# leimao/Voice-Converter-CycleGAN

Hardware: NVIDIA H100
Metric: CycleGAN-VC train steps/sec @ batch 256x[24,128] MCEP (higher is better)
Workload: dtype f16f8 (forward / data gradient: fp16 MMA + two e4m3 cross-term MMAs = 2 MMA units per product; weight gradient: fp16 MMA alone, 1 unit; f32 accumulate)

## Files before the change

voice-converter-cyclegan_b200/csrc/tc_gemm.cu:

```cuda
#include "tc_gemm.cuh"
#include "geom.h"
#include "kernels.cuh"
#include "wgmma.cuh"

#include <cuda.h>
#include <stdint.h>
#include <stdio.h>
#include <string.h>

namespace {

typedef CUresult (*EncodeTiledFn)(CUtensorMap*, CUtensorMapDataType, cuuint32_t, void*, const cuuint64_t*, const cuuint64_t*,
                                  const cuuint32_t*, const cuuint32_t*, CUtensorMapInterleave, CUtensorMapSwizzle,
                                  CUtensorMapL2promotion, CUtensorMapFloatOOBfill);
EncodeTiledFn get_encoder() {
  static EncodeTiledFn fn = nullptr;
  if (!fn) {
    void* p = nullptr; cudaDriverEntryPointQueryResult q;
    if (cudaGetDriverEntryPoint("cuTensorMapEncodeTiled", &p, cudaEnableDefault, &q) == cudaSuccess && q == cudaDriverEntryPointSuccess)
      fn = (EncodeTiledFn)p;
  }
  return fn;
}
bool make_tmap3(CUtensorMap* m, const void* base, uint64_t d0, uint64_t d1, uint64_t d2, uint32_t b1) {
  EncodeTiledFn enc = get_encoder();
  if (!enc) return false;
  cuuint64_t dims[3] = {d0, d1, d2};
  cuuint64_t strides[2] = {d0 * 2, d0 * d1 * 2};
  cuuint32_t box[3] = {64, b1, 1};
  cuuint32_t es[3] = {1, 1, 1};
  return enc(m, CU_TENSOR_MAP_DATA_TYPE_BFLOAT16, 3, const_cast<void*>(base), dims, strides, box, es, CU_TENSOR_MAP_INTERLEAVE_NONE,
             CU_TENSOR_MAP_SWIZZLE_128B, CU_TENSOR_MAP_L2_PROMOTION_L2_256B, CU_TENSOR_MAP_FLOAT_OOB_FILL_NONE) == CUDA_SUCCESS;
}

bool make_tmap3_t(CUtensorMap* m, const void* base, CUtensorMapDataType dt, int esize, uint64_t d0, uint64_t d1, uint64_t d2, uint32_t b0, uint32_t b1) {
  EncodeTiledFn enc = get_encoder();
  if (!enc) return false;
  cuuint64_t dims[3] = {d0, d1, d2};
  cuuint64_t strides[2] = {d0 * (uint64_t)esize, d0 * d1 * (uint64_t)esize};
  cuuint32_t box[3] = {b0, b1, 1};
  cuuint32_t es[3] = {1, 1, 1};
  return enc(m, dt, 3, const_cast<void*>(base), dims, strides, box, es, CU_TENSOR_MAP_INTERLEAVE_NONE,
             b0 * esize == 64 ? CU_TENSOR_MAP_SWIZZLE_64B : CU_TENSOR_MAP_SWIZZLE_128B, CU_TENSOR_MAP_L2_PROMOTION_L2_256B,
             CU_TENSOR_MAP_FLOAT_OOB_FILL_NONE) == CUDA_SUCCESS;
}

__device__ __forceinline__ uint32_t smem_u32(const void* p) { return (uint32_t)__cvta_generic_to_shared(p); }

__device__ __forceinline__ void mbar_init(uint64_t* bar, uint32_t count) {
  asm volatile("mbarrier.init.shared::cta.b64 [%0], %1;" ::"r"(smem_u32(bar)), "r"(count));
}
__device__ __forceinline__ void fence_barrier_init() { asm volatile("fence.mbarrier_init.release.cluster;" ::: "memory"); }
__device__ __forceinline__ void mbar_wait(uint64_t* bar, uint32_t parity) {
  asm volatile(
      "{\n\t"
      ".reg .pred p;\n\t"
      "WAIT_LOOP:\n\t"
      "mbarrier.try_wait.parity.shared::cta.b64 p, [%0], %1;\n\t"
      "@p bra.uni WAIT_DONE;\n\t"
      "bra.uni WAIT_LOOP;\n\t"
      "WAIT_DONE:\n\t"
      "}" ::"r"(smem_u32(bar)), "r"(parity) : "memory");
}
__device__ __forceinline__ void cp_async16(uint32_t dst_smem, const void* src, uint32_t src_bytes) {
  asm volatile("cp.async.cg.shared.global [%0], [%1], 16, %2;" ::"r"(dst_smem), "l"(src), "r"(src_bytes) : "memory");
}
__device__ __forceinline__ void cp_async_arrive_noinc(uint64_t* bar) {
  asm volatile("cp.async.mbarrier.arrive.noinc.shared::cta.b64 [%0];" ::"r"(smem_u32(bar)) : "memory");
}
__device__ __forceinline__ void mbar_expect_tx(uint64_t* bar, uint32_t bytes) {
  asm volatile("mbarrier.arrive.expect_tx.shared::cta.b64 _, [%0], %1;" ::"r"(smem_u32(bar)), "r"(bytes) : "memory");
}
__device__ __forceinline__ void tma_load3(uint32_t dst_smem, const CUtensorMap* map, int c0, int c1, int c2, uint64_t* bar) {
  asm volatile("cp.async.bulk.tensor.3d.shared::cluster.global.tile.mbarrier::complete_tx::bytes [%0], [%1, {%2, %3, %4}], [%5];"
               ::"r"(dst_smem), "l"(map), "r"(c0), "r"(c1), "r"(c2), "r"(smem_u32(bar)) : "memory");
}
__device__ __forceinline__ void tma_prefetch_desc(const CUtensorMap* map) {
  asm volatile("prefetch.tensormap [%0];" ::"l"(map) : "memory");
}
__device__ __forceinline__ void fence_proxy_async() { asm volatile("fence.proxy.async.shared::cta;" ::: "memory"); }
__device__ __forceinline__ uint64_t make_desc(uint32_t smem_addr, uint32_t lbo_bytes, uint32_t sbo_bytes, uint64_t layout = 1) {
  return (uint64_t)((smem_addr >> 4) & 0x3FFF) | ((uint64_t)((lbo_bytes >> 4) & 0x3FFF) << 16) |
         ((uint64_t)((sbo_bytes >> 4) & 0x3FFF) << 32) | (layout << 62);
}
__device__ __forceinline__ uint64_t make_desc64(uint32_t smem_addr) { return make_desc(smem_addr, 16, 512, 2); }
template <int N>
__device__ __forceinline__ void fence_acc(float (&d)[N]) {
#pragma unroll
  for (int i = 0; i < N; ++i) asm volatile("" : "+f"(d[i])::"memory");
}
__device__ __forceinline__ void mbar_arrive(uint64_t* bar) {
  asm volatile("mbarrier.arrive.shared::cta.b64 _, [%0];" ::"r"(smem_u32(bar)) : "memory");
}
__device__ __forceinline__ void consumer_bar() { asm volatile("bar.sync 3, 256;" ::: "memory"); }
__device__ __forceinline__ void st_shared16(uint32_t addr, uint4 v) {
  asm volatile("st.shared.v4.b32 [%0], {%1, %2, %3, %4};" ::"r"(addr), "r"(v.x), "r"(v.y), "r"(v.z), "r"(v.w) : "memory");
}
__device__ __forceinline__ uint4 e4m3x8_to_f16x8(uint2 v) {
  uint32_t w[4];
#pragma unroll
  for (int i = 0; i < 4; ++i) {
    const uint32_t src = (i < 2 ? v.x : v.y) >> (16 * (i & 1));
    const __half2_raw h = __nv_cvt_fp8x2_to_halfraw2((__nv_fp8x2_storage_t)(src & 0xFFFFu), __NV_E4M3);
    w[i] = (uint32_t)h.x | ((uint32_t)h.y << 16);
  }
  return make_uint4(w[0], w[1], w[2], w[3]);
}

struct FastDiv { uint32_t mul, shr, d; };
__host__ inline FastDiv make_fastdiv(uint32_t d) {
  FastDiv f; f.d = d;
  uint32_t l = 0; while ((1ull << l) < d) ++l;
  f.mul = (uint32_t)(((1ull << 32) * ((1ull << l) - d)) / d + 1);
  f.shr = l;
  return f;
}
__device__ __forceinline__ uint32_t fdiv(uint32_t n, const FastDiv& f) { return (uint32_t)(((uint64_t)__umulhi(n, f.mul) + n) >> f.shr); }

__device__ __forceinline__ uint32_t sw128(int r, int c) { return (uint32_t)((r >> 3) * 1024 + (r & 7) * 128 + ((c ^ (r & 7)) << 4)); }

struct TcNTParams {
  GatherGeom g;
  const __nv_bfloat16 *a_hi, *a_lo; int a_ld; int C;
  const __nv_bfloat16 *b_hi, *b_lo; int Nw;
  int N;
  int n_tiles;
  int debug;
  float* dst; int d_ld; const float* bias; int accumulate;
  int perm; int Cc;
  int R;
  const float *gamma_a, *beta_a, *gamma_g, *beta_g;
  float* stats;
  const float* resid;
  float* y; __nv_bfloat16 *y_hi, *y_lo;
  int C_out;
  const float* bp; int bp_ld;
  __nv_bfloat16 *dp_hi, *dp_lo; int dp_ld;
  float *dbeta_a, *dgamma_a, *dbeta_g, *dgamma_g;
  CUtensorMap tm_b_hi, tm_b_lo;
  const uint8_t *a8_hi, *a8_lo;
  CUtensorMap tm_b8_hi, tm_b8_lo;
  uint8_t* y8;
  PackGeom pk;
  FastDiv div_bw, div_w;
};

struct RowPos { int b, y, x; };
__device__ __forceinline__ RowPos nt_row(const TcNTParams& p, long long m) {
  RowPos r;
  r.y = (int)fdiv((uint32_t)m, p.div_bw);
  const uint32_t rem = (uint32_t)m - (uint32_t)r.y * p.div_bw.d;
  r.b = (int)fdiv(rem, p.div_w);
  r.x = (int)(rem - (uint32_t)r.b * p.div_w.d);
  return r;
}
template <int PK = 0>
__device__ __forceinline__ uint32_t nt_tile_taps(const TcNTParams& p, long long m0, long long M) {
  const long long m1 = m0 + 127 < M ? m0 + 127 : M - 1;
  if constexpr (PK == 2) {
    const int dout = p.pk.div * p.g.sx;
    const Pack2Pos a = pack2_pos(p.pk, p.g.Hy, dout, m0), b = pack2_pos(p.pk, p.g.Hy, dout, m1);
    return a.u == b.u ? gather_tap_mask(p.g, a.y, b.y) : (1u << p.g.ntaps) - 1u;
  }
  return gather_tap_mask(p.g, nt_row(p, m0).y, nt_row(p, m1).y);
}

struct TcTNParams {
  GatherGeom g;
  const __nv_bfloat16 *x_hi, *x_lo; int x_ld; int C;
  const __nv_bfloat16 *g_hi, *g_lo; int g_ld; int N;
  float* dw_a; float* dw_g; int n_split;
  int ksplit;
  FastDiv div_hw, div_w;
  CUtensorMap tm_g_hi, tm_g_lo;
  const uint8_t *x8_hi, *x8_lo;
  const uint8_t *g8_hi, *g8_lo;
  int w16;
  int fold_n;
  float* part; long long part_k, numel_a;
  PackGeom pk;
};

__device__ __forceinline__ float* tn_dst(float* base, int slab, int C, int c, int ncols, int col, int fold_n) {
  if (fold_n) { const int t = col / fold_n; return base + ((long long)t * C + c) * fold_n + (col - t * fold_n); }
  return base + ((long long)slab * C + c) * ncols + col;
}

constexpr int kProducerThreads = 128;


template <int BN, int NPL>
struct NTCfg {
  static constexpr int A_PLANE = 128 * 128;
  static constexpr int B_PLANE = BN * 128;
  static constexpr int PLANES = NPL == 2 ? 2 : 1;
  static constexpr int STAGE = PLANES * (A_PLANE + B_PLANE);
  static constexpr int STAGES = (192 * 1024) / STAGE;
  static constexpr int SMEM = STAGES * STAGE + 1024;
// ... 394 lines not shown
        }
        float t[32];
#pragma unroll
        for (int k = 0; k < 32; ++k) t[k] = dy[k];
        float s1a = warp_colsum32(t, lane);
#pragma unroll
        for (int k = 0; k < 32; ++k) t[k] = dy[k] * xa[k];
        float s2a = warp_colsum32(t, lane);
        float s1g = 0.f, s2g = 0.f;
        if (EPI == 3) {
#pragma unroll
          for (int k = 0; k < 32; ++k) t[k] = dg[k];
          s1g = warp_colsum32(t, lane);
#pragma unroll
          for (int k = 0; k < 32; ++k) t[k] = dg[k] * xg[k];
          s2g = warp_colsum32(t, lane);
        }
        if (p.dbeta_a && live) {
          atomicAdd(p.dbeta_a + ch + lane, s1a); atomicAdd(p.dgamma_a + ch + lane, s2a);
          if (EPI == 3) { atomicAdd(p.dbeta_g + ch + lane, s1g); atomicAdd(p.dgamma_g + ch + lane, s2g); }
        }
        s1a = sample_sum(s1a, epi_xch, q, lane, spw, barid); s2a = sample_sum(s2a, epi_xch, q, lane, spw, barid);
        if (EPI == 3) { s1g = sample_sum(s1g, epi_xch, q, lane, spw, barid); s2g = sample_sum(s2g, epi_xch, q, lane, spw, barid); }
        {
          const float sca = bc[64 + lane], scg = EPI == 3 ? bc[192 + lane] : 0.f;
          __syncwarp();
          bc[256 + lane] = sca * s1a * invR; bc[288 + lane] = sca * s2a * invR;
          if (EPI == 3) { bc[320 + lane] = scg * s1g * invR; bc[352 + lane] = scg * s2g * invR; }
          __syncwarp();
        }
#pragma unroll
        for (int k = 0; k < 32; k += 4) {
          float c1[4], c2[4], c3[4];
          bc4(bc + 64 + k, c1); bc4(bc + 256 + k, c2); bc4(bc + 288 + k, c3);
#pragma unroll
          for (int j = 0; j < 4; ++j) dy[k + j] = fmaf(c1[j], dy[k + j], -fmaf(xa[k + j], c3[j], c2[j]));
        }
        hwrite_y(stg, dy, nullptr, p.dp_hi, p.dp_lo, mq, M, p.dp_ld, ch, lane);
        if (EPI == 3) {
#pragma unroll
          for (int k = 0; k < 32; k += 4) {
            float c1[4], c2[4], c3[4];
            bc4(bc + 192 + k, c1); bc4(bc + 320 + k, c2); bc4(bc + 352 + k, c3);
#pragma unroll
            for (int j = 0; j < 4; ++j) dg[k + j] = fmaf(c1[j], dg[k + j], -fmaf(xg[k + j], c3[j], c2[j]));
          }
          hwrite_y(stg, dg, nullptr, p.dp_hi, p.dp_lo, mq, M, p.dp_ld, C + ch, lane);
        }
      }
    }
  }
}

enum { MMA_BF16 = 0, MMA_BF16X3 = 1, MMA_E4M3_CROSS = 2, MMA_F16 = 3, MMA_F16_CROSS = 4 };

template <int BN, int KIND, int TN, class Cfg>
__device__ __forceinline__ void consume_stages(float (&d)[BN / 2], int nkb, int& stage, uint32_t& phase, int& prev,
                                               uint64_t* full_bar, uint64_t* empty_bar, uint32_t smem_base, int wg, int lane) {
  for (int kb = 0; kb < nkb; ++kb) {
    mbar_wait(&full_bar[stage], phase);
    fence_proxy_async();
    const uint32_t sA = smem_base + stage * Cfg::STAGE + wg * 8192;
    const uint32_t sB = smem_base + stage * Cfg::STAGE + Cfg::PLANES * Cfg::A_PLANE;
    fence_acc(d);
    wgmma_fence();
    if constexpr (TN == 0) {
      if constexpr (KIND == MMA_E4M3_CROSS) {
#pragma unroll
        for (int k = 0; k < 2; ++k) {
          wgmma_e4m3<BN>(d, make_desc(sA + k * 32, 16, 1024), make_desc64(sB + Cfg::B_PLANE / 2 + k * 32), 1);
          wgmma_e4m3<BN>(d, make_desc(sA + 64 + k * 32, 16, 1024), make_desc64(sB + k * 32), 1);
        }
      } else if constexpr (KIND == MMA_F16) {
#pragma unroll
        for (int k = 0; k < 4; ++k)
          wgmma_f16<BN, 0, 0>(d, make_desc(sA + k * 32, 16, 1024), make_desc(sB + k * 32, 16, 1024), 1);
      } else {
#pragma unroll
        for (int k = 0; k < 4; ++k) {
          const uint64_t a_hi = make_desc(sA + k * 32, 16, 1024), b_hi = make_desc(sB + k * 32, 16, 1024);
          wgmma_bf16<BN, 0, 0>(d, a_hi, b_hi, 1);
          if constexpr (KIND == MMA_BF16X3) {
            const uint64_t a_lo = make_desc(sA + Cfg::A_PLANE + k * 32, 16, 1024), b_lo = make_desc(sB + Cfg::B_PLANE + k * 32, 16, 1024);
            wgmma_bf16<BN, 0, 0>(d, a_hi, b_lo, 1);
            wgmma_bf16<BN, 0, 0>(d, a_lo, b_hi, 1);
          }
        }
      }
    } else {
#pragma unroll
      for (int k = 0; k < 4; ++k) {
        const uint64_t a0 = make_desc(sA + k * 2048, 8192, 1024), b0 = make_desc(sB + k * 2048, 8192, 1024);
        const uint64_t a1 = make_desc(sA + Cfg::A_PLANE + k * 2048, 8192, 1024), b1 = make_desc(sB + Cfg::B_PLANE + k * 2048, 8192, 1024);
        if constexpr (KIND == MMA_F16_CROSS) {
          wgmma_f16<BN, 1, 1>(d, a0, b1, 1);
          wgmma_f16<BN, 1, 1>(d, a1, b0, 1);
        } else if constexpr (KIND == MMA_F16) {
          wgmma_f16<BN, 1, 1>(d, a0, b0, 1);
        } else {
          wgmma_bf16<BN, 1, 1>(d, a0, b0, 1);
          if constexpr (KIND == MMA_BF16X3) {
            wgmma_bf16<BN, 1, 1>(d, a0, b1, 1);
            wgmma_bf16<BN, 1, 1>(d, a1, b0, 1);
          }
        }
      }
    }
    wgmma_commit();
    wgmma_wait<1>();
    fence_acc(d);
    if (prev >= 0 && lane == 0) mbar_arrive(&empty_bar[prev]);
    prev = stage;
    if (++stage == Cfg::STAGES) { stage = 0; phase ^= 1; }
  }
}
template <int N>
__device__ __forceinline__ void rescale_acc(float (&d)[N], float scale) {
  wgmma_wait<0>();
  fence_acc(d);
#pragma unroll
  for (int i = 0; i < N; ++i) d[i] *= scale;
}

template <int BN, int PK = 0>
__device__ __forceinline__ void nt_store_fragments(const TcNTParams& p, const float (&d)[BN / 2], const long long M,
                                                   const long long m0, const int n0, const int r, const int c) {
  const GatherGeom& g = p.g;
  float* rowp[2];
#pragma unroll
  for (int h = 0; h < 2; ++h) {
    const long long m = m0 + r + 8 * h;
    rowp[h] = nullptr;
    if (m < M && p.dst) {
      if constexpr (PK == 2) {
        const int dout = p.pk.div * g.sx;
        const Pack2Pos o = pack2_pos(p.pk, g.Hy, dout, m);
        const long long r = pack2_row(o.o0, o.o1, g.Hd, dout / g.dsx, o.y * g.dsy + g.doy, o.x * g.dsx + g.dox);
        if (r >= 0) rowp[h] = p.dst + r * p.d_ld;
      } else {
        const RowPos o = nt_row(p, m);
        rowp[h] = p.dst + ((long long)(o.b * g.Hd + o.y * g.dsy + g.doy) * g.Wd + o.x * g.dsx + g.dox) * p.d_ld;
      }
    }
  }
  const bool vec = (p.d_ld & 1) == 0;
#pragma unroll
  for (int j = 0; j < BN / 8; ++j) {
    const int cb = j >> 2;
    const int n = (p.perm == 2 ? (cb >> 2) * p.Cc + ((cb >> 1) & 1) * (p.Cc >> 1) + (n0 >> 2) + (cb & 1) * 32
                   : p.perm    ? ((cb < 4) ? (n0 >> 1) + cb * 32 : p.Cc + (n0 >> 1) + (cb - 4) * 32) : n0 + cb * 32) + ((8 * j) & 31) + c;
    if (n >= p.N) continue;
    float2 bb = make_float2(0.f, 0.f);
    if (p.bias) bb = *reinterpret_cast<const float2*>(p.bias + n0 + 8 * j + c);
#pragma unroll
    for (int h = 0; h < 2; ++h) {
      float* rp = rowp[h];
      if (rp == nullptr) continue;
      float v0 = d[4 * j + 2 * h], v1 = d[4 * j + 2 * h + 1];
      if (p.bias) { v0 += bb.x; v1 += bb.y; }
      if (vec && n + 2 <= p.N) {
        if (p.accumulate)
          asm volatile("red.global.add.v2.f32 [%0], {%1, %2};" ::"l"(rp + n), "f"(v0), "f"(v1) : "memory");
        else
          *reinterpret_cast<float2*>(rp + n) = make_float2(v0, v1);
      } else {
        if (p.accumulate) atomicAdd(rp + n, v0); else rp[n] = v0;
        if (n + 1 < p.N) { if (p.accumulate) atomicAdd(rp + n + 1, v1); else rp[n + 1] = v1; }
      }
    }
  }
}

constexpr int kNTThreads = 384;

template <int BN, int NPL, int EPI, int PK = 0>
__global__ void __launch_bounds__(kNTThreads, 1)
tc_gg_nt_kernel(const __grid_constant__ TcNTParams p) {
  static_assert(!PK || EPI == 0, "packed rows never take the fused epilogues (they need whole equal-length samples per tile)");
  using Cfg = NTCfg<BN, NPL>;
  __shared__ float epi_xch[2][4][32];
  __shared__ __align__(16) float epi_bc[8][(EPI == 3 || EPI == 4) ? 384 : 128];
  __shared__ __align__(16) float epi_stage[8][32 * 16];
  __shared__ float* epi_rowp[8][32];
  constexpr int S = Cfg::STAGES;
  extern __shared__ uint8_t smem_raw[];
  __shared__ __align__(8) uint64_t full_bar[S], empty_bar[S], acc_free_bar;

  const uint32_t smem_base = (smem_u32(smem_raw) + 1023u) & ~1023u;
  const int warp = threadIdx.x >> 5, lane = threadIdx.x & 31;
  const GatherGeom& g = p.g;
  const long long M = (long long)g.B * g.Hy * g.Wx;
  const int cchunks = p.C >> 6;
  const int m_tiles = (int)((M + 127) / 128);
  const int n_tiles = p.n_tiles;
  const int num_tiles = m_tiles * n_tiles;
  const bool n_fast = g.Hy > 1;

  if (threadIdx.x == 0) {
    for (int s = 0; s < S; ++s) { mbar_init(&full_bar[s], kProducerThreads + 1); mbar_init(&empty_bar[s], 8); }
    mbar_init(&acc_free_bar, 8);
    fence_barrier_init();
    tma_prefetch_desc(&p.tm_b_hi);
    if (NPL == 2) tma_prefetch_desc(&p.tm_b_lo);
    if (NPL == 3) { tma_prefetch_desc(&p.tm_b8_hi); tma_prefetch_desc(&p.tm_b8_lo); }
  }
  __syncthreads();

  if (warp < 4) {
    const int t = threadIdx.x;
    const int chunk = t & 7, rsub = t >> 3;
    int stage = 0; uint32_t phase = 0;
    int it = 0;
    for (int tile = blockIdx.x; tile < num_tiles; tile += gridDim.x, ++it) {
      const long long m0 = (long long)(n_fast ? tile / n_tiles : tile % m_tiles) * 128;
      const int n0 = (n_fast ? tile % n_tiles : tile / m_tiles) * BN;
      if (EPI != 0 && it > 0) mbar_wait(&acc_free_bar, (uint32_t)(it - 1) & 1u);
      const uint32_t taps = nt_tile_taps<PK>(p, m0, M);
      int rb[8], ry[8], rx[8];
      int rw[PK == 2 ? 8 : 1];
#pragma unroll
      for (int i = 0; i < 8; ++i) {
        long long m = m0 + rsub + 16 * i;
        if (m < M) {
          if constexpr (PK == 2) {
            const Pack2Pos o = pack2_pos(p.pk, g.Hy, p.pk.div * g.sx, m);
            rb[i] = (int)(g.Hs * o.o0 / p.pk.div); rw[i] = (int)((o.o1 - o.o0) / p.pk.div); ry[i] = o.y * g.sy; rx[i] = o.x * g.sx;
          } else if constexpr (PK) {
            const int dout = p.pk.div * g.sx;
            const int u = pack_find(p.pk.off, p.pk.n, m * dout);
            const long long o0 = __ldg(p.pk.off + u), o1 = __ldg(p.pk.off + u + 1);
            rb[i] = (int)(o0 / p.pk.div); ry[i] = (int)((o1 - o0) / p.pk.div); rx[i] = (int)(m - o0 / dout) * g.sx;
          } else {
            const RowPos o = nt_row(p, m);
            rb[i] = o.b; ry[i] = o.y * g.sy; rx[i] = o.x * g.sx;
          }
        } else { rb[i] = -1; ry[i] = 0; rx[i] = 0; }
      }
      for (int pass = 0; pass < (NPL == 3 ? 2 : 1); ++pass)
      for (int tap = 0; tap < g.ntaps; ++tap) {
        if (!((taps >> tap) & 1u)) continue;
        long long aoff[8];
#pragma unroll
        for (int i = 0; i < 8; ++i) {
          const int cofs = NPL == 3 && pass == 0 ? (chunk & 3) * 16 : chunk * 8;
          if constexpr (PK == 2) {
            const int yy = ry[i] + g.oy[tap], xx = rx[i] + g.ox[tap];
            aoff[i] = rb[i] >= 0 && yy >= 0 && yy < g.Hs && xx >= 0 && xx < rw[i] ? ((long long)rb[i] + yy * rw[i] + xx) * p.a_ld + cofs : -1;
          } else if constexpr (PK) {
            const int xx = rx[i] + g.ox[tap];
            aoff[i] = rb[i] >= 0 && xx >= 0 && xx < ry[i] ? (long long)(rb[i] + xx) * p.a_ld + cofs : -1;
          } else {
            int yy = ry[i] + g.oy[tap], xx = rx[i] + g.ox[tap];
            bool ok = rb[i] >= 0 && yy >= 0 && yy < g.Hs && xx >= 0 && xx < g.Ws;
            aoff[i] = ok ? ((long long)(rb[i] * g.Hs + yy) * g.Ws + xx) * p.a_ld + cofs : -1;
          }
        }
        for (int cc = 0; cc < cchunks; ++cc) {
          const int c0 = cc << 6;
          mbar_wait(&empty_bar[stage], phase ^ 1);
          const uint32_t sA = smem_base + stage * Cfg::STAGE;
          const uint32_t sB = sA + Cfg::PLANES * Cfg::A_PLANE;
          if (t == 0) {
            mbar_expect_tx(&full_bar[stage], Cfg::PLANES * Cfg::B_PLANE);
            if (NPL == 3) {
              if (pass == 0) {
                tma_load3(sB, &p.tm_b8_hi, c0, n0, g.widx[tap], &full_bar[stage]);
                tma_load3(sB + Cfg::B_PLANE / 2, &p.tm_b8_lo, c0, n0, g.widx[tap], &full_bar[stage]);
              } else {
                tma_load3(sB, &p.tm_b_hi, c0, n0, g.widx[tap], &full_bar[stage]);
              }
            } else {
              tma_load3(sB, &p.tm_b_hi, c0, n0, g.widx[tap], &full_bar[stage]);
              if (NPL == 2) tma_load3(sB + Cfg::B_PLANE, &p.tm_b_lo, c0, n0, g.widx[tap], &full_bar[stage]);
            }
          }
          if (!(p.debug & 4)) {
#pragma unroll
            for (int i = 0; i < 8; ++i) {
              const int r = rsub + 16 * i;
              const uint32_t so = sw128(r, chunk);
              const bool ok = aoff[i] >= 0;
              const long long off = ok ? aoff[i] + c0 : 0;
              if (NPL == 3) {
                if (pass == 0)
                  cp_async16(sA + so, (chunk < 4 ? p.a8_hi : p.a8_lo) + off, ok ? 16u : 0u);
                else
                  cp_async16(sA + so, p.a_hi + off, ok ? 16u : 0u);
              } else {
                cp_async16(sA + so, p.a_hi + off, ok ? 16u : 0u);
                if (NPL == 2) cp_async16(sA + Cfg::A_PLANE + so, p.a_lo + off, ok ? 16u : 0u);
              }
            }
          }
          cp_async_arrive_noinc(&full_bar[stage]);
          if (++stage == S) { stage = 0; phase ^= 1; }
        }
      }
    }
  } else {
    const int cw = warp - 4;
    const int wg = cw >> 2;
    const int tw = threadIdx.x - 128 * (wg + 1);
    float* acc_s = reinterpret_cast<float*>(smem_raw + (smem_base - smem_u32(smem_raw)));
    int stage = 0; uint32_t phase = 0;
    for (int tile = blockIdx.x; tile < num_tiles; tile += gridDim.x) {
      const long long m0 = (long long)(n_fast ? tile / n_tiles : tile % m_tiles) * 128;
      const int n0 = (n_fast ? tile % n_tiles : tile / m_tiles) * BN;
      float d[BN / 2];
#pragma unroll
      for (int i = 0; i < BN / 2; ++i) d[i] = 0.f;
      int prev = -1;
      const int kb_pass = __popc(nt_tile_taps<PK>(p, m0, M)) * cchunks;
      if constexpr (NPL == 3) {
        consume_stages<BN, MMA_E4M3_CROSS, 0, Cfg>(d, kb_pass, stage, phase, prev, full_bar, empty_bar, smem_base, wg, lane);
        rescale_acc(d, 1.f / (float)(1 << CGVC_Q_ACC_SHIFT));
        consume_stages<BN, MMA_F16, 0, Cfg>(d, kb_pass, stage, phase, prev, full_bar, empty_bar, smem_base, wg, lane);
      } else {
        consume_stages<BN, NPL == 2 ? MMA_BF16X3 : MMA_BF16, 0, Cfg>(d, kb_pass, stage, phase, prev, full_bar, empty_bar, smem_base, wg, lane);
      }
      wgmma_wait<0>();
      fence_acc(d);
      if (prev >= 0 && lane == 0) mbar_arrive(&empty_bar[prev]);
      const int r0 = wg * 64 + (tw >> 5) * 16 + ((tw & 31) >> 2), c0 = 2 * (tw & 3);
      if constexpr (EPI == 0) {
        if (!(p.debug & 3)) nt_store_fragments<BN, PK>(p, d, M, m0, n0, r0, c0);
      } else {
        consumer_bar();
        if (!(p.debug & 2)) {
#pragma unroll
          for (int j = 0; j < BN / 8; ++j) {
            *reinterpret_cast<float2*>(acc_s + acc_off<BN>(r0, 8 * j + c0)) = make_float2(d[4 * j], d[4 * j + 1]);
            *reinterpret_cast<float2*>(acc_s + acc_off<BN>(r0 + 8, 8 * j + c0)) = make_float2(d[4 * j + 2], d[4 * j + 3]);
          }
        }
        consumer_bar();
        nt_tile_epilogue<BN, NPL, EPI>(p, M, m0, n0, cw & 3, lane, epi_stage[cw], epi_rowp[cw], epi_bc[cw], epi_xch[wg], acc_s, wg, 2);
        fence_proxy_async();
        __syncwarp();
        if (lane == 0) mbar_arrive(&acc_free_bar);
      }
    }
  }
}

#define CGVC_Q_WGRAD_SHIFT 12
template <int NPL, int W16>
struct TNCfg {
  static constexpr int A_PLANE = 64 * 256;
  static constexpr int B_PLANE = 64 * 512;
  static constexpr int PLANES = (NPL == 1 || W16) ? 1 : 2;
  static constexpr int STAGE = PLANES * (A_PLANE + B_PLANE);
  static constexpr int STAGES = (192 * 1024) / STAGE;
  static constexpr int SMEM = STAGES * STAGE + 1024;
};

template <int NPL, int W16, int DET, int PK = 0>
__global__ void __launch_bounds__(kNTThreads, 1)
tc_gg_tn_kernel(const __grid_constant__ TcTNParams p) {
  static_assert(W16 == 0 || NPL == 3, "the fp16-only weight gradient is a form of CGVC_PREC_F16F8");
  using Cfg = TNCfg<NPL, W16>;
  constexpr int S = Cfg::STAGES;
  constexpr int BN = 256;
  extern __shared__ uint8_t smem_raw[];
  __shared__ __align__(8) uint64_t full_bar[S], empty_bar[S];

  const uint32_t smem_base = (smem_u32(smem_raw) + 1023u) & ~1023u;
  const int warp = threadIdx.x >> 5, lane = threadIdx.x & 31;
// ... 302 lines not shown
  {
    const int lane = t & 31, warp = t >> 5;
    const int cig = (lane & 3) * 8;
    const int col = warp * 8 + (lane >> 2);
    const int co = co0 + col;
    if (co < J.cout && ci0 + cig < J.cin_q) {
      float va[4], vb[4];
#pragma unroll
      for (int k = 0; k < 4; ++k) { va[k] = tile[cig + k][col]; vb[k] = tile[cig + 4 + k][col]; }
      const int nrow = perm_row(J.perm, co, J.cout, J.noff);
      const long long o = ((long long)tap * J.nt_n + nrow) * J.cin_q + ci0 + cig;
      uint2 ha, hb; uint32_t a_hi, a_lo, b_hi, b_lo;
      cgvc_quant4(va, CGVC_Q_W_SHI, CGVC_Q_W_SLO, ha, a_hi, a_lo);
      cgvc_quant4(vb, CGVC_Q_W_SHI, CGVC_Q_W_SLO, hb, b_hi, b_lo);
      *reinterpret_cast<uint4*>(J.q16 + o) = make_uint4(ha.x, ha.y, hb.x, hb.y);
      *reinterpret_cast<uint2*>(J.q8hi + o) = make_uint2(a_hi, b_hi);
      *reinterpret_cast<uint2*>(J.q8lo + o) = make_uint2(a_lo, b_lo);
    }
  }
  if (tap == 0 && tci == 0 && tco == 0 && J.b_off >= 0)
    for (int i = t; i < J.cout; i += 256) J.bias[perm_row(J.perm, i, J.cout, J.noff)] = params[J.b_off + i];
}

template <class K>
cudaError_t set_smem(K kernel, int bytes) {
  static std::vector<const void*> done;
  const void* key = (const void*)kernel;
  for (const void* d : done) if (d == key) return cudaSuccess;
  cudaError_t e = cudaFuncSetAttribute(kernel, cudaFuncAttributeMaxDynamicSharedMemorySize, bytes);
  if (e == cudaSuccess) done.push_back(key);
  return e;
}

struct ProfRec { cudaEvent_t a, b; double flops; int cls; long long M; int N, K; };
bool g_prof_on = false;
std::vector<ProfRec> g_prof;
void prof_begin(cudaStream_t st, double flops, int cls, long long M = 0, int N = 0, int K = 0) {
  if (!g_prof_on) return;
  ProfRec r; r.flops = flops; r.cls = cls; r.M = M; r.N = N; r.K = K;
  cudaEventCreate(&r.a); cudaEventCreate(&r.b);
  cudaEventRecord(r.a, st);
  g_prof.push_back(r);
}
void prof_end(cudaStream_t st) { if (g_prof_on && !g_prof.empty()) cudaEventRecord(g_prof.back().b, st); }

inline int tile_rows(int n_real, int n_padded) { return (n_padded % 256 == 0) ? 256 : (n_real <= 32 ? 32 : 128); }

int num_sms() {
  static int n = 0;
  if (!n) { int dev = 0; cudaGetDevice(&dev); cudaDeviceGetAttribute(&n, cudaDevAttrMultiProcessorCount, dev); }
  return n;
}

cudaError_t launch_nt(TcNTParams p, int precision, cudaStream_t st, int epi) {
  const long long M = (long long)p.g.B * p.g.Hy * p.g.Wx;
  if (M == 0) return cudaSuccess;
  if (M >= (1ll << 31)) return cudaErrorInvalidValue;
  const bool x3 = precision == 1;
  if (p.g.ntaps == 0) return cudaErrorInvalidValue;
  p.div_bw = make_fastdiv((uint32_t)(p.g.B * p.g.Wx)); p.div_w = make_fastdiv((uint32_t)p.g.Wx);
  const int bn = tile_rows(p.N, p.Nw);
  p.n_tiles = bn == 32 ? 1 : p.Nw / bn;
  const long long tiles = ((M + 127) / 128) * p.n_tiles;
  dim3 grid((unsigned)(tiles < num_sms() ? tiles : num_sms()));
  cudaError_t e;
  ++g_cgvc_launches;
  prof_begin(st, 2.0 * (double)M * p.N * p.g.ntaps * p.C, (epi == 1 || epi == 2 || epi == 5) ? 2 : 0, M, p.N, p.g.ntaps * p.C);
#define LAUNCH_NT(BN_, NPL_, EPI_, ...)                                                                        \
  do {                                                                                                         \
    e = set_smem(tc_gg_nt_kernel<BN_, NPL_, EPI_, ##__VA_ARGS__>, NTCfg<BN_, NPL_>::SMEM);                     \
    if (e != cudaSuccess) return e;                                                                            \
    tc_gg_nt_kernel<BN_, NPL_, EPI_, ##__VA_ARGS__><<<grid, kNTThreads, NTCfg<BN_, NPL_>::SMEM, st>>>(p);      \
  } while (0)
  if (epi != 0 && bn != 256) return cudaErrorInvalidValue;
  if (p.pk.off && (p.g.Hy > 1 || p.g.Hs > 1 || p.g.Hd > 1)) {
    if (epi != 0 || p.g.B != 1 || p.g.ntaps > 31) return cudaErrorInvalidValue;
    const int npl = precision == 3 ? 3 : x3 ? 2 : 1;
    if (bn == 256)      { if (npl == 3) LAUNCH_NT(256, 3, 0, 2); else if (npl == 2) LAUNCH_NT(256, 2, 0, 2); else LAUNCH_NT(256, 1, 0, 2); }
    else if (bn == 128) { if (npl == 3) LAUNCH_NT(128, 3, 0, 2); else if (npl == 2) LAUNCH_NT(128, 2, 0, 2); else LAUNCH_NT(128, 1, 0, 2); }
    else                { if (npl == 3) LAUNCH_NT(32, 3, 0, 2);  else if (npl == 2) LAUNCH_NT(32, 2, 0, 2);  else LAUNCH_NT(32, 1, 0, 2); }
  }
  else if (p.pk.off) {
    if (epi != 0 || p.g.B != 1 || p.g.Hy != 1) return cudaErrorInvalidValue;
    const int npl = precision == 3 ? 3 : x3 ? 2 : 1;
    if (bn == 256)      { if (npl == 3) LAUNCH_NT(256, 3, 0, 1); else if (npl == 2) LAUNCH_NT(256, 2, 0, 1); else LAUNCH_NT(256, 1, 0, 1); }
    else if (bn == 128) { if (npl == 3) LAUNCH_NT(128, 3, 0, 1); else if (npl == 2) LAUNCH_NT(128, 2, 0, 1); else LAUNCH_NT(128, 1, 0, 1); }
    else                { if (npl == 3) LAUNCH_NT(32, 3, 0, 1);  else if (npl == 2) LAUNCH_NT(32, 2, 0, 1);  else LAUNCH_NT(32, 1, 0, 1); }
  }
  else if (precision == 3) {
    if (epi == 1)       LAUNCH_NT(256, 3, 1);
    else if (epi == 2)  LAUNCH_NT(256, 3, 2);
    else if (epi == 5)  LAUNCH_NT(256, 3, 5);
    else if (epi != 0)  return cudaErrorInvalidValue;
    else if (bn == 256) LAUNCH_NT(256, 3, 0);
    else if (bn == 128) LAUNCH_NT(128, 3, 0);
    else                LAUNCH_NT(32, 3, 0);
  }
  else if (epi == 1)  { if (x3) LAUNCH_NT(256, 2, 1); else LAUNCH_NT(256, 1, 1); }
  else if (epi == 2)  { if (x3) LAUNCH_NT(256, 2, 2); else LAUNCH_NT(256, 1, 2); }
  else if (epi == 3)  { if (x3) LAUNCH_NT(256, 2, 3); else LAUNCH_NT(256, 1, 3); }
  else if (epi == 4)  { if (x3) LAUNCH_NT(256, 2, 4); else LAUNCH_NT(256, 1, 4); }
  else if (epi == 5)  { if (x3) LAUNCH_NT(256, 2, 5); else LAUNCH_NT(256, 1, 5); }
  else if (bn == 256) { if (x3) LAUNCH_NT(256, 2, 0); else LAUNCH_NT(256, 1, 0); }
  else if (bn == 128) { if (x3) LAUNCH_NT(128, 2, 0); else LAUNCH_NT(128, 1, 0); }
  else                { if (x3) LAUNCH_NT(32, 2, 0);  else LAUNCH_NT(32, 1, 0); }
#undef LAUNCH_NT
  prof_end(st);
  return cudaGetLastError();
}

cudaError_t launch_tn(TcTNParams p, int precision, cudaStream_t st, const DetSlab* det) {
  const long long M = (long long)p.g.B * p.g.Hy * p.g.Wx;
  if (M == 0) return cudaSuccess;
  if (M >= (1ll << 31)) return cudaErrorInvalidValue;
  const int tiles = ((p.g_ld + 255) / 256) * ((p.x_ld + 127) / 128) * p.g.ntaps;
  const int nsm = num_sms();
  long long maxsplit = M / 1024; if (maxsplit < 1) maxsplit = 1; if (maxsplit > 32) maxsplit = 32;
  int ksplit = 1; double best = 0.0;
  for (int ks = 1; ks <= (int)maxsplit; ++ks) {
    long long items = (long long)tiles * ks;
    double eff = (double)items / (double)(((items + nsm - 1) / nsm) * nsm);
    if (items < nsm) eff *= 0.5;
    if (eff > best + 0.02) { best = eff; ksplit = ks; }
  }
  const long long numel = (long long)p.g.ntaps * p.C * p.N;
  auto chunk_of = [&](int ks) { return ((M + ks - 1) / ks + 63) / 64 * 64; };
  if (det && det->p)
    while (ksplit > 1 && ((long long)ksplit * numel > det->cap || (long long)(ksplit - 1) * chunk_of(ksplit) >= M)) --ksplit;
  const bool det_split = det && det->p && ksplit > 1;
  if (det_split) { p.part = det->p; p.part_k = numel; p.numel_a = (long long)p.g.ntaps * p.C * p.n_split; }
  p.ksplit = ksplit;
  p.div_hw = make_fastdiv((uint32_t)(p.g.Hy * p.g.Wx)); p.div_w = make_fastdiv((uint32_t)p.g.Wx);
  const long long items = (long long)tiles * ksplit;
  dim3 grid((unsigned)(items < nsm ? items : nsm));
  cudaError_t e;
  ++g_cgvc_launches;
  prof_begin(st, 2.0 * (double)M * p.N * p.g.ntaps * p.C, 1, M, p.N, p.g.ntaps * p.C);
#define LAUNCH_TN(NPL_, W16_, DET_, ...)                                                                      \
  do {                                                                                                        \
    e = set_smem(tc_gg_tn_kernel<NPL_, W16_, DET_, ##__VA_ARGS__>, TNCfg<NPL_, W16_>::SMEM);                  \
    if (e != cudaSuccess) return e;                                                                           \
    tc_gg_tn_kernel<NPL_, W16_, DET_, ##__VA_ARGS__><<<grid, kNTThreads, TNCfg<NPL_, W16_>::SMEM, st>>>(p);   \
  } while (0)
  if (p.pk.off && (p.g.Hy > 1 || p.g.Hs > 1)) {
    if (p.g.B != 1) return cudaErrorInvalidValue;
    if (det_split) {
      if (precision == 3) { if (p.w16) LAUNCH_TN(3, 1, 1, 2); else LAUNCH_TN(3, 0, 1, 2); }
      else if (precision == 1) LAUNCH_TN(2, 0, 1, 2);
      else                     LAUNCH_TN(1, 0, 1, 2);
    } else {
      if (precision == 3) { if (p.w16) LAUNCH_TN(3, 1, 0, 2); else LAUNCH_TN(3, 0, 0, 2); }
      else if (precision == 1) LAUNCH_TN(2, 0, 0, 2);
      else                     LAUNCH_TN(1, 0, 0, 2);
    }
  } else if (p.pk.off) {
    if (p.g.B != 1 || p.g.Hy != 1) return cudaErrorInvalidValue;
    if (det_split) {
      if (precision == 3) { if (p.w16) LAUNCH_TN(3, 1, 1, 1); else LAUNCH_TN(3, 0, 1, 1); }
// ... 231 lines not shown
    L.bias = (float*)p; p += rnd((size_t)nt_n(L) * sizeof(float));
    if (!make_layer_maps(L)) return (int)cudaErrorInvalidValue;
    L.wq16 = nullptr; L.wq8hi = L.wq8lo = nullptr; L.wdq16 = nullptr; L.wdq8hi = L.wdq8lo = nullptr;
    if (w.quant && layer_ok_q(L)) {
      L.wq16 = p; p += rnd(wq_elems(L) * 2);
      L.wq8hi = (uint8_t*)p; p += rnd(wq_elems(L)); L.wq8lo = (uint8_t*)p; p += rnd(wq_elems(L));
      if (w.quant_bwd) {
        L.wdq16 = p; p += rnd(wdq_elems(L) * 2);
        L.wdq8hi = (uint8_t*)p; p += rnd(wdq_elems(L)); L.wdq8lo = (uint8_t*)p; p += rnd(wdq_elems(L));
      }
      if (!make_layer_maps_q(L)) return (int)cudaErrorInvalidValue;
    }
  }
  w.job_first.clear(); w.job_ka.clear();
  if (w.quant) {
    std::vector<PrepJob> jobs;
    int blocks = 0;
    for (TcLayer& L : w.layers) {
      if (!L.wq16) continue;
      for (int br = 0; br < (L.gated ? 2 : 1); ++br) {
        PrepJob J; memset(&J, 0, sizeof J);
        J.w_off = (long long)(br ? L.kg : L.ka); J.b_off = L.fold ? -1 : (long long)(br ? L.bg : L.ba);
        J.taps = L.kh * L.kw; J.cin = L.cin; J.cout = L.cout; J.nt_n = nt_n(L); J.cin_q = cin_q(L); J.cin_n = cin_n(L); J.nt_q = nt_q(L);
        J.noff = br ? L.cout : 0; J.perm = layer_perm(L); J.fold_n = L.fold ? L.cout / L.fold : 0;
        J.q16 = (__half*)L.wq16; J.q8hi = L.wq8hi; J.q8lo = L.wq8lo;
        J.dq16 = (__half*)L.wdq16; J.dq8hi = L.wdq8hi; J.dq8lo = L.wdq8lo;
        J.bias = L.bias;
        J.tiles_ci = (L.cin + 31) / 32; J.tiles_co = (L.cout + 63) / 64;
        J.first_block = blocks;
        blocks += J.taps * J.tiles_ci * J.tiles_co;
        jobs.push_back(J); w.job_first.push_back(J.first_block); w.job_ka.push_back(L.ka);
      }
    }
    w.job_first.push_back(blocks);
    if (!jobs.empty()) {
      err = cudaMalloc(&w.prep_jobs, jobs.size() * sizeof(PrepJob));
      if (err != cudaSuccess) return (int)err;
      err = cudaMemcpy(w.prep_jobs, jobs.data(), jobs.size() * sizeof(PrepJob), cudaMemcpyHostToDevice);
      if (err != cudaSuccess) return (int)err;
    }
  }
  w.ready = false;
  return 0;
}

static cudaError_t tc_init_kernels() {
  cudaError_t e;
#define INIT_NT(BN_, NPL_, EPI_) if ((e = set_smem(tc_gg_nt_kernel<BN_, NPL_, EPI_>, NTCfg<BN_, NPL_>::SMEM)) != cudaSuccess) return e;
  INIT_NT(256, 2, 0) INIT_NT(256, 1, 0) INIT_NT(128, 2, 0) INIT_NT(128, 1, 0) INIT_NT(32, 2, 0) INIT_NT(32, 1, 0)
  INIT_NT(256, 2, 1) INIT_NT(256, 1, 1) INIT_NT(256, 2, 2) INIT_NT(256, 1, 2)
  INIT_NT(256, 2, 3) INIT_NT(256, 1, 3) INIT_NT(256, 2, 4) INIT_NT(256, 1, 4) INIT_NT(256, 2, 5) INIT_NT(256, 1, 5)
  INIT_NT(256, 3, 0) INIT_NT(128, 3, 0) INIT_NT(32, 3, 0) INIT_NT(256, 3, 1) INIT_NT(256, 3, 2) INIT_NT(256, 3, 5)
#undef INIT_NT
#define INIT_NT_PK(BN_, NPL_, PK_) if ((e = set_smem(tc_gg_nt_kernel<BN_, NPL_, 0, PK_>, NTCfg<BN_, NPL_>::SMEM)) != cudaSuccess) return e;
  INIT_NT_PK(256, 1, 1) INIT_NT_PK(256, 2, 1) INIT_NT_PK(256, 3, 1) INIT_NT_PK(128, 1, 1) INIT_NT_PK(128, 2, 1) INIT_NT_PK(128, 3, 1)
  INIT_NT_PK(32, 1, 1) INIT_NT_PK(32, 2, 1) INIT_NT_PK(32, 3, 1)
  INIT_NT_PK(256, 1, 2) INIT_NT_PK(256, 2, 2) INIT_NT_PK(256, 3, 2) INIT_NT_PK(128, 1, 2) INIT_NT_PK(128, 2, 2) INIT_NT_PK(128, 3, 2)
  INIT_NT_PK(32, 1, 2) INIT_NT_PK(32, 2, 2) INIT_NT_PK(32, 3, 2)
#undef INIT_NT_PK
#define INIT_TN(NPL_, W16_, DET_) if ((e = set_smem(tc_gg_tn_kernel<NPL_, W16_, DET_>, TNCfg<NPL_, W16_>::SMEM)) != cudaSuccess) return e;
  INIT_TN(3, 1, 0) INIT_TN(3, 0, 0) INIT_TN(2, 0, 0) INIT_TN(1, 0, 0)
  INIT_TN(3, 1, 1) INIT_TN(3, 0, 1) INIT_TN(2, 0, 1) INIT_TN(1, 0, 1)
#define INIT_TN_PK(NPL_, W16_, DET_, PK_) if ((e = set_smem(tc_gg_tn_kernel<NPL_, W16_, DET_, PK_>, TNCfg<NPL_, W16_>::SMEM)) != cudaSuccess) return e;
  INIT_TN_PK(3, 1, 0, 1) INIT_TN_PK(3, 0, 0, 1) INIT_TN_PK(2, 0, 0, 1) INIT_TN_PK(1, 0, 0, 1)
  INIT_TN_PK(3, 1, 1, 1) INIT_TN_PK(3, 0, 1, 1) INIT_TN_PK(2, 0, 1, 1) INIT_TN_PK(1, 0, 1, 1)
  INIT_TN_PK(3, 1, 0, 2) INIT_TN_PK(3, 0, 0, 2) INIT_TN_PK(2, 0, 0, 2) INIT_TN_PK(1, 0, 0, 2)
  INIT_TN_PK(3, 1, 1, 2) INIT_TN_PK(3, 0, 1, 2) INIT_TN_PK(2, 0, 1, 2) INIT_TN_PK(1, 0, 1, 2)
#undef INIT_TN_PK
#undef INIT_TN
  return cudaSuccess;
}

void tc_free(TcWeights& w) {
  if (w.pool) cudaFree(w.pool);
  if (w.prep_jobs) cudaFree(w.prep_jobs);
  w.pool = nullptr; w.prep_jobs = nullptr; w.ready = false;
}

static int refresh_jobs(TcWeights& w, const float* params, int j0, int j1, cudaStream_t st) {
  if (j1 <= j0) return 0;
  const int b0 = w.job_first[j0], nb = w.job_first[j1] - b0;
  ++g_cgvc_launches;
  prep_weights_q_all_kernel<<<(unsigned)nb, 256, 0, st>>>(params, (const PrepJob*)w.prep_jobs, j0, j1, b0);
  return (int)cudaGetLastError();
}

int tc_refresh_weights(TcWeights& w, const float* params, cudaStream_t st) {
  if (!w.pool) return 0;
  const bool batched = w.prep_batched && w.prep_jobs;
  for (TcLayer& L : w.layers) {
    if (batched && L.wq16) continue;
    int r = tc_refresh_layer(L, params + L.ka, params + L.kg, params + L.ba, params + L.bg, st);
    if (r != 0) return r;
  }
  if (batched) { int r = refresh_jobs(w, params, 0, (int)w.job_ka.size(), st); if (r != 0) return r; }
  w.ready = true;
  return 0;
}

int tc_refresh_weights_range(TcWeights& w, const float* params, size_t begin, size_t end, cudaStream_t st) {
  if (!w.pool) return 0;
  const bool batched = w.prep_batched && w.prep_jobs;
  for (TcLayer& L : w.layers) {
    if (L.ka < begin || L.ka >= end) continue;
    if (batched && L.wq16) continue;
    int r = tc_refresh_layer(L, params + L.ka, params + L.kg, params + L.ba, params + L.bg, st);
// ... 76 lines not shown
```

Baseline: 10.01.

## Load NT GEMM activation tiles with 4D TMA instead of cp.async gather

Adds 4D tensor maps over the activation tensor, using element strides to express the conv stride, so a single producer thread issues TMA loads for the A operand instead of 128 threads doing cp.async gathers. A new e4m3 cross MMA variant handles the 64B-swizzled fp8 layout that TMA produces. The goal is to free producer warps from address arithmetic and per-thread copies and to reduce load-issue overhead. The fast path only applies when the geometry fits (width divides 128, stride at most 8) and falls back otherwise. The risk is layout or descriptor mismatches, and a larger parameter struct.

```diff
diff --git a/voice-converter-cyclegan_b200/csrc/tc_gemm.cu b/voice-converter-cyclegan_b200/csrc/tc_gemm.cu
--- a/voice-converter-cyclegan_b200/csrc/tc_gemm.cu
+++ b/voice-converter-cyclegan_b200/csrc/tc_gemm.cu
@@ -42,6 +42,18 @@
   cuuint32_t es[3] = {1, 1, 1};
   return enc(m, dt, 3, const_cast<void*>(base), dims, strides, box, es, CU_TENSOR_MAP_INTERLEAVE_NONE,
              b0 * esize == 64 ? CU_TENSOR_MAP_SWIZZLE_64B : CU_TENSOR_MAP_SWIZZLE_128B, CU_TENSOR_MAP_L2_PROMOTION_L2_256B,
+             CU_TENSOR_MAP_FLOAT_OOB_FILL_NONE) == CUDA_SUCCESS;
+}
+
+bool make_tmap_act(CUtensorMap* m, const void* base, int esize, uint64_t ld, const GatherGeom& g, uint32_t bx, uint32_t nb) {
+  EncodeTiledFn enc = get_encoder();
+  if (!enc) return false;
+  cuuint64_t dims[4] = {ld, (cuuint64_t)g.Ws, (cuuint64_t)g.Hs, (cuuint64_t)g.B};
+  cuuint64_t strides[3] = {ld * esize, ld * esize * g.Ws, ld * esize * g.Ws * g.Hs};
+  cuuint32_t box[4] = {64, bx, 1, nb};
+  cuuint32_t es[4] = {1, (cuuint32_t)g.sx, 1, 1};
+  return enc(m, esize == 1 ? CU_TENSOR_MAP_DATA_TYPE_UINT8 : CU_TENSOR_MAP_DATA_TYPE_UINT16, 4, const_cast<void*>(base), dims, strides, box, es,
+             CU_TENSOR_MAP_INTERLEAVE_NONE, esize == 1 ? CU_TENSOR_MAP_SWIZZLE_64B : CU_TENSOR_MAP_SWIZZLE_128B, CU_TENSOR_MAP_L2_PROMOTION_L2_256B,
              CU_TENSOR_MAP_FLOAT_OOB_FILL_NONE) == CUDA_SUCCESS;
 }
 
@@ -74,6 +86,10 @@
 __device__ __forceinline__ void tma_load3(uint32_t dst_smem, const CUtensorMap* map, int c0, int c1, int c2, uint64_t* bar) {
   asm volatile("cp.async.bulk.tensor.3d.shared::cluster.global.tile.mbarrier::complete_tx::bytes [%0], [%1, {%2, %3, %4}], [%5];"
                ::"r"(dst_smem), "l"(map), "r"(c0), "r"(c1), "r"(c2), "r"(smem_u32(bar)) : "memory");
+}
+__device__ __forceinline__ void tma_load4(uint32_t dst_smem, const CUtensorMap* map, int c0, int c1, int c2, int c3, uint64_t* bar) {
+  asm volatile("cp.async.bulk.tensor.4d.shared::cluster.global.tile.mbarrier::complete_tx::bytes [%0], [%1, {%2, %3, %4, %5}], [%6];"
+               ::"r"(dst_smem), "l"(map), "r"(c0), "r"(c1), "r"(c2), "r"(c3), "r"(smem_u32(bar)) : "memory");
 }
 __device__ __forceinline__ void tma_prefetch_desc(const CUtensorMap* map) {
   asm volatile("prefetch.tensormap [%0];" ::"l"(map) : "memory");
@@ -143,7 +159,9 @@
   uint8_t* y8;
   PackGeom pk;
   FastDiv div_bw, div_w;
+  CUtensorMap tm_a_hi, tm_a_lo, tm_a8_hi, tm_a8_lo;
 };
+static_assert(sizeof(TcNTParams) <= 4096, "kernel parameters are limited to 4 KB");
 
 struct RowPos { int b, y, x; };
 __device__ __forceinline__ RowPos nt_row(const TcNTParams& p, long long m) {
@@ -644,7 +662,7 @@
   }
 }
 
-enum { MMA_BF16 = 0, MMA_BF16X3 = 1, MMA_E4M3_CROSS = 2, MMA_F16 = 3, MMA_F16_CROSS = 4 };
+enum { MMA_BF16 = 0, MMA_BF16X3 = 1, MMA_E4M3_CROSS = 2, MMA_F16 = 3, MMA_F16_CROSS = 4, MMA_E4M3_CROSS64 = 5 };
 
 template <int BN, int KIND, int TN, class Cfg>
 __device__ __forceinline__ void consume_stages(float (&d)[BN / 2], int nkb, int& stage, uint32_t& phase, int& prev,
@@ -652,7 +670,7 @@
   for (int kb = 0; kb < nkb; ++kb) {
     mbar_wait(&full_bar[stage], phase);
     fence_proxy_async();
-    const uint32_t sA = smem_base + stage * Cfg::STAGE + wg * 8192;
+    const uint32_t sA = smem_base + stage * Cfg::STAGE + wg * (KIND == MMA_E4M3_CROSS64 ? 4096 : 8192);
     const uint32_t sB = smem_base + stage * Cfg::STAGE + Cfg::PLANES * Cfg::A_PLANE;
     fence_acc(d);
     wgmma_fence();
@@ -662,6 +680,12 @@
         for (int k = 0; k < 2; ++k) {
           wgmma_e4m3<BN>(d, make_desc(sA + k * 32, 16, 1024), make_desc64(sB + Cfg::B_PLANE / 2 + k * 32), 1);
           wgmma_e4m3<BN>(d, make_desc(sA + 64 + k * 32, 16, 1024), make_desc64(sB + k * 32), 1);
+        }
+      } else if constexpr (KIND == MMA_E4M3_CROSS64) {
+#pragma unroll
+        for (int k = 0; k < 2; ++k) {
+          wgmma_e4m3<BN>(d, make_desc64(sA + k * 32), make_desc64(sB + Cfg::B_PLANE / 2 + k * 32), 1);
+          wgmma_e4m3<BN>(d, make_desc64(sA + Cfg::A_PLANE / 2 + k * 32), make_desc64(sB + k * 32), 1);
         }
       } else if constexpr (KIND == MMA_F16) {
 #pragma unroll
@@ -765,10 +789,11 @@
 
 constexpr int kNTThreads = 384;
 
-template <int BN, int NPL, int EPI, int PK = 0>
+template <int BN, int NPL, int EPI, int PK = 0, int TA = 0>
 __global__ void __launch_bounds__(kNTThreads, 1)
 tc_gg_nt_kernel(const __grid_constant__ TcNTParams p) {
   static_assert(!PK || EPI == 0, "packed rows never take the fused epilogues (they need whole equal-length samples per tile)");
+  static_assert(!PK || !TA, "the TMA form is dense");
   using Cfg = NTCfg<BN, NPL>;
   __shared__ float epi_xch[2][4][32];
   __shared__ __align__(16) float epi_bc[8][(EPI == 3 || EPI == 4) ? 384 : 128];
@@ -789,16 +814,62 @@
   const bool n_fast = g.Hy > 1;
 
   if (threadIdx.x == 0) {
-    for (int s = 0; s < S; ++s) { mbar_init(&full_bar[s], kProducerThreads + 1); mbar_init(&empty_bar[s], 8); }
+    for (int s = 0; s < S; ++s) { mbar_init(&full_bar[s], TA ? 1 : kProducerThreads + 1); mbar_init(&empty_bar[s], 8); }
     mbar_init(&acc_free_bar, 8);
     fence_barrier_init();
     tma_prefetch_desc(&p.tm_b_hi);
     if (NPL == 2) tma_prefetch_desc(&p.tm_b_lo);
     if (NPL == 3) { tma_prefetch_desc(&p.tm_b8_hi); tma_prefetch_desc(&p.tm_b8_lo); }
+    if (TA) {
+      tma_prefetch_desc(&p.tm_a_hi);
+      if (NPL == 2) tma_prefetch_desc(&p.tm_a_lo);
+      if (NPL == 3) { tma_prefetch_desc(&p.tm_a8_hi); tma_prefetch_desc(&p.tm_a8_lo); }
+    }
   }
   __syncthreads();
 
-  if (warp < 4) {
+  if (TA && warp < 4) {
+    if (threadIdx.x == 0) {
+      int stage = 0; uint32_t phase = 0;
+      int it = 0;
+      for (int tile = blockIdx.x; tile < num_tiles; tile += gridDim.x, ++it) {
+        const long long m0 = (long long)(n_fast ? tile / n_tiles : tile % m_tiles) * 128;
+        const int n0 = (n_fast ? tile % n_tiles : tile / m_tiles) * BN;
+        if (EPI != 0 && it > 0) mbar_wait(&acc_free_bar, (uint32_t)(it - 1) & 1u);
+        const uint32_t taps = nt_tile_taps<PK>(p, m0, M);
+        const RowPos o = nt_row(p, m0);
+        const uint32_t a_bytes = (p.debug & 4) ? 0u : (uint32_t)Cfg::PLANES * Cfg::A_PLANE;
+        for (int pass = 0; pass < (NPL == 3 ? 2 : 1); ++pass)
+        for (int tap = 0; tap < g.ntaps; ++tap) {
+          if (!((taps >> tap) & 1u)) continue;
+          const int xs = o.x * g.sx + g.ox[tap], ys = o.y * g.sy + g.oy[tap];
+          for (int cc = 0; cc < cchunks; ++cc) {
+            const int c0 = cc << 6;
+            mbar_wait(&empty_bar[stage], phase ^ 1);
+            const uint32_t sA = smem_base + stage * Cfg::STAGE;
+            const uint32_t sB = sA + Cfg::PLANES * Cfg::A_PLANE;
+            mbar_expect_tx(&full_bar[stage], a_bytes + Cfg::PLANES * Cfg::B_PLANE);
+            if (NPL == 3 && pass == 0) {
+              tma_load3(sB, &p.tm_b8_hi, c0, n0, g.widx[tap], &full_bar[stage]);
+              tma_load3(sB + Cfg::B_PLANE / 2, &p.tm_b8_lo, c0, n0, g.widx[tap], &full_bar[stage]);
+              if (a_bytes) {
+                tma_load4(sA, &p.tm_a8_hi, c0, xs, ys, o.b, &full_bar[stage]);
+                tma_load4(sA + Cfg::A_PLANE / 2, &p.tm_a8_lo, c0, xs, ys, o.b, &full_bar[stage]);
+              }
+            } else {
+              tma_load3(sB, &p.tm_b_hi, c0, n0, g.widx[tap], &full_bar[stage]);
+              if (NPL == 2) tma_load3(sB + Cfg::B_PLANE, &p.tm_b_lo, c0, n0, g.widx[tap], &full_bar[stage]);
+              if (a_bytes) {
+                tma_load4(sA, &p.tm_a_hi, c0, xs, ys, o.b, &full_bar[stage]);
+                if (NPL == 2) tma_load4(sA + Cfg::A_PLANE, &p.tm_a_lo, c0, xs, ys, o.b, &full_bar[stage]);
+              }
+            }
+            if (++stage == S) { stage = 0; phase ^= 1; }
+          }
+        }
+      }
+    }
+  } else if (warp < 4) {
     const int t = threadIdx.x;
     const int chunk = t & 7, rsub = t >> 3;
     int stage = 0; uint32_t phase = 0;
@@ -904,7 +975,7 @@
       int prev = -1;
       const int kb_pass = __popc(nt_tile_taps<PK>(p, m0, M)) * cchunks;
       if constexpr (NPL == 3) {
-        consume_stages<BN, MMA_E4M3_CROSS, 0, Cfg>(d, kb_pass, stage, phase, prev, full_bar, empty_bar, smem_base, wg, lane);
+        consume_stages<BN, TA ? MMA_E4M3_CROSS64 : MMA_E4M3_CROSS, 0, Cfg>(d, kb_pass, stage, phase, prev, full_bar, empty_bar, smem_base, wg, lane);
         rescale_acc(d, 1.f / (float)(1 << CGVC_Q_ACC_SHIFT));
         consume_stages<BN, MMA_F16, 0, Cfg>(d, kb_pass, stage, phase, prev, full_bar, empty_bar, smem_base, wg, lane);
       } else {
@@ -1313,6 +1384,17 @@
   return n;
 }
 
+static bool nt_tma_maps(TcNTParams& p, int npl) {
+  const GatherGeom& g = p.g;
+  const int wx = g.Wx < 128 ? g.Wx : 128;
+  if (128 % wx || g.Wx % wx || (g.Hy > 1 && ((long long)g.B * g.Wx) % 128) || wx * g.sx > 256 || g.sx > 8) return false;
+  const uint32_t bx = (uint32_t)(wx * g.sx), nb = (uint32_t)(128 / wx);
+  if (npl == 3)
+    return make_tmap_act(&p.tm_a_hi, p.a_hi, 2, p.a_ld, g, bx, nb) && make_tmap_act(&p.tm_a8_hi, p.a8_hi, 1, p.a_ld, g, bx, nb) &&
+           make_tmap_act(&p.tm_a8_lo, p.a8_lo, 1, p.a_ld, g, bx, nb);
+  return make_tmap_act(&p.tm_a_hi, p.a_hi, 2, p.a_ld, g, bx, nb) && (npl != 2 || make_tmap_act(&p.tm_a_lo, p.a_lo, 2, p.a_ld, g, bx, nb));
+}
+
 cudaError_t launch_nt(TcNTParams p, int precision, cudaStream_t st, int epi) {
   const long long M = (long long)p.g.B * p.g.Hy * p.g.Wx;
   if (M == 0) return cudaSuccess;
@@ -1348,23 +1430,28 @@
     else if (bn == 128) { if (npl == 3) LAUNCH_NT(128, 3, 0, 1); else if (npl == 2) LAUNCH_NT(128, 2, 0, 1); else LAUNCH_NT(128, 1, 0, 1); }
     else                { if (npl == 3) LAUNCH_NT(32, 3, 0, 1);  else if (npl == 2) LAUNCH_NT(32, 2, 0, 1);  else LAUNCH_NT(32, 1, 0, 1); }
   }
-  else if (precision == 3) {
-    if (epi == 1)       LAUNCH_NT(256, 3, 1);
-    else if (epi == 2)  LAUNCH_NT(256, 3, 2);
-    else if (epi == 5)  LAUNCH_NT(256, 3, 5);
-    else if (epi != 0)  return cudaErrorInvalidValue;
-    else if (bn == 256) LAUNCH_NT(256, 3, 0);
-    else if (bn == 128) LAUNCH_NT(128, 3, 0);
-    else                LAUNCH_NT(32, 3, 0);
-  }
-  else if (epi == 1)  { if (x3) LAUNCH_NT(256, 2, 1); else LAUNCH_NT(256, 1, 1); }
-  else if (epi == 2)  { if (x3) LAUNCH_NT(256, 2, 2); else LAUNCH_NT(256, 1, 2); }
-  else if (epi == 3)  { if (x3) LAUNCH_NT(256, 2, 3); else LAUNCH_NT(256, 1, 3); }
-  else if (epi == 4)  { if (x3) LAUNCH_NT(256, 2, 4); else LAUNCH_NT(256, 1, 4); }
-  else if (epi == 5)  { if (x3) LAUNCH_NT(256, 2, 5); else LAUNCH_NT(256, 1, 5); }
-  else if (bn == 256) { if (x3) LAUNCH_NT(256, 2, 0); else LAUNCH_NT(256, 1, 0); }
-  else if (bn == 128) { if (x3) LAUNCH_NT(128, 2, 0); else LAUNCH_NT(128, 1, 0); }
-  else                { if (x3) LAUNCH_NT(32, 2, 0);  else LAUNCH_NT(32, 1, 0); }
+  else {
+    const bool ta = nt_tma_maps(p, precision == 3 ? 3 : x3 ? 2 : 1);
+#define LAUNCH_NT_D(BN_, NPL_, EPI_) do { if (ta) LAUNCH_NT(BN_, NPL_, EPI_, 0, 1); else LAUNCH_NT(BN_, NPL_, EPI_); } while (0)
+    if (precision == 3) {
+      if (epi == 1)       LAUNCH_NT_D(256, 3, 1);
+      else if (epi == 2)  LAUNCH_NT_D(256, 3, 2);
+      else if (epi == 5)  LAUNCH_NT_D(256, 3, 5);
+      else if (epi != 0)  return cudaErrorInvalidValue;
+      else if (bn == 256) LAUNCH_NT_D(256, 3, 0);
+      else if (bn == 128) LAUNCH_NT_D(128, 3, 0);
+      else                LAUNCH_NT_D(32, 3, 0);
+    }
+    else if (epi == 1)  { if (x3) LAUNCH_NT_D(256, 2, 1); else LAUNCH_NT_D(256, 1, 1); }
+    else if (epi == 2)  { if (x3) LAUNCH_NT_D(256, 2, 2); else LAUNCH_NT_D(256, 1, 2); }
+    else if (epi == 3)  { if (x3) LAUNCH_NT_D(256, 2, 3); else LAUNCH_NT_D(256, 1, 3); }
+    else if (epi == 4)  { if (x3) LAUNCH_NT_D(256, 2, 4); else LAUNCH_NT_D(256, 1, 4); }
+    else if (epi == 5)  { if (x3) LAUNCH_NT_D(256, 2, 5); else LAUNCH_NT_D(256, 1, 5); }
+    else if (bn == 256) { if (x3) LAUNCH_NT_D(256, 2, 0); else LAUNCH_NT_D(256, 1, 0); }
+    else if (bn == 128) { if (x3) LAUNCH_NT_D(128, 2, 0); else LAUNCH_NT_D(128, 1, 0); }
+    else                { if (x3) LAUNCH_NT_D(32, 2, 0);  else LAUNCH_NT_D(32, 1, 0); }
+#undef LAUNCH_NT_D
+  }
 #undef LAUNCH_NT
   prof_end(st);
   return cudaGetLastError();
@@ -1702,6 +1789,12 @@
   INIT_NT(256, 2, 3) INIT_NT(256, 1, 3) INIT_NT(256, 2, 4) INIT_NT(256, 1, 4) INIT_NT(256, 2, 5) INIT_NT(256, 1, 5)
   INIT_NT(256, 3, 0) INIT_NT(128, 3, 0) INIT_NT(32, 3, 0) INIT_NT(256, 3, 1) INIT_NT(256, 3, 2) INIT_NT(256, 3, 5)
 #undef INIT_NT
+#define INIT_NT(BN_, NPL_, EPI_) if ((e = set_smem(tc_gg_nt_kernel<BN_, NPL_, EPI_, 0, 1>, NTCfg<BN_, NPL_>::SMEM)) != cudaSuccess) return e;
+  INIT_NT(256, 2, 0) INIT_NT(256, 1, 0) INIT_NT(128, 2, 0) INIT_NT(128, 1, 0) INIT_NT(32, 2, 0) INIT_NT(32, 1, 0)
+  INIT_NT(256, 2, 1) INIT_NT(256, 1, 1) INIT_NT(256, 2, 2) INIT_NT(256, 1, 2)
+  INIT_NT(256, 2, 3) INIT_NT(256, 1, 3) INIT_NT(256, 2, 4) INIT_NT(256, 1, 4) INIT_NT(256, 2, 5) INIT_NT(256, 1, 5)
+  INIT_NT(256, 3, 0) INIT_NT(128, 3, 0) INIT_NT(32, 3, 0) INIT_NT(256, 3, 1) INIT_NT(256, 3, 2) INIT_NT(256, 3, 5)
+#undef INIT_NT
 #define INIT_NT_PK(BN_, NPL_, PK_) if ((e = set_smem(tc_gg_nt_kernel<BN_, NPL_, 0, PK_>, NTCfg<BN_, NPL_>::SMEM)) != cudaSuccess) return e;
   INIT_NT_PK(256, 1, 1) INIT_NT_PK(256, 2, 1) INIT_NT_PK(256, 3, 1) INIT_NT_PK(128, 1, 1) INIT_NT_PK(128, 2, 1) INIT_NT_PK(128, 3, 1)
   INIT_NT_PK(32, 1, 1) INIT_NT_PK(32, 2, 1) INIT_NT_PK(32, 3, 1)
```

Measured after the change: 10.77 (median of 6 runs). +7.5%, better.
